# hsinnan75/GSAlign

Hardware: AMD Instinct MI355X
Metric: aligned query Gbp/s (whole node) (higher is better)
Workload: dtype u8; 1 GPU; full-human-sized pair (BASELINE configs[4]): 24 contigs with GRCh38 chromosome lengths, 3.08 Gbp, repeat injection, vs 1; inflight_contexts_per_gpu=8, world_size=1, parallelism=one GPU

## Files before the change

### gsalign_amd/csrc/gsa_api.hip

```cpp
#include <algorithm>
#include <atomic>
#include <chrono>
#include <cstring>
#include <mutex>
#include <thread>
#include <pthread.h>
#include <sched.h>
#include "gsa_ctx.h"

static thread_local std::string g_create_error;

int gsa_fail(gsa_ctx *ctx, int code, const std::string &msg)
{
	if (ctx) ctx->err = msg; else g_create_error = msg;
	return code;
}

int host_stage4_5_6(gsa_ctx *c, int stage);
int host_stage8_finish(gsa_ctx *c);
int build_block_view(gsa_ctx *c);
void bundle_split_lists(gsa_ctx *c);
void bundle_join_lists(gsa_ctx *c);

void collect_events(gsa_ctx *c)
// ... 418 lines not shown
	return GSA_OK;
}

int gsa_set_option(gsa_ctx *c, const char *name, int64_t value)
{
	if (!c || !name) return GSA_ERR_ARG;
	const std::string k(name);
	auto in = [&](int64_t lo, int64_t hi) { return value >= lo && value <= hi; };
	const int64_t BIG = (int64_t)1 << 40;
	if (k == "split_min") { if (!in(0, BIG)) return gsa_fail(c, GSA_ERR_ARG, "split_min: 0 .. 2^40 bases"); c->opt.split_min = value; }
	else if (k == "bundle_contig") { if (!in(0, BIG)) return gsa_fail(c, GSA_ERR_ARG, "bundle_contig: 0 (no bundles) .. 2^40 bases"); c->opt.bundle_contig = value; }
	else if (k == "bundle_cap") { if (!in(1, BIG)) return gsa_fail(c, GSA_ERR_ARG, "bundle_cap: 1 .. 2^40 bases"); c->opt.bundle_cap = value; }
	else if (k == "seed_budget") { if (!in(1, 0xffffffffll)) return gsa_fail(c, GSA_ERR_ARG, "seed_budget: 1 .. 2^32 - 1 wave-iterations"); c->seed_budget = (u32)value; }
	else if (k == "dp_lane") { if (!in(0, 1 << 20)) return gsa_fail(c, GSA_ERR_ARG, "dp_lane: 0 (round 2's tiny / small split) .. 2^20 cells"); c->opt.dp_lane = (int)value; }
	else if (k == "seed_mode") { if (value < 0 || value > 2) return gsa_fail(c, GSA_ERR_ARG, "seed_mode: 0 sweep, 1 speculative, 2 search"); c->opt.seed_mode = (int)value; }
	else if (k == "pd_bitmap") c->opt.pd_bitmap = value != 0;
	else if (k == "dp_side") c->opt.dp_side = value != 0;
	else if (k == "dp_small_side") c->opt.dp_small_side = value != 0;
	else if (k == "pd_two_level_min") { if (!in(0, BIG)) return gsa_fail(c, GSA_ERR_ARG, "pd_two_level_min: >= 0 blocks"); c->opt.pd_two_level_min = value; }
	else if (k == "dp_occupancy") { if (!in(0, 16)) return gsa_fail(c, GSA_ERR_ARG, "dp_occupancy: 0 (off) .. 16 workgroups per CU"); c->opt.dp_occupancy = (int)value; }
	else if (k == "pd_bytes") { if (!in(0, 2)) return gsa_fail(c, GSA_ERR_ARG, "pd_bytes: 0 never, 1 by the hit count, 2 always"); c->opt.pd_bytes = (int)value; }
	else if (k == "pres_from_kmer") c->opt.pres_from_kmer = value != 0;
	else if (k == "walk_chain_min") { if (!in(0, BIG)) return gsa_fail(c, GSA_ERR_ARG, "walk_chain_min: >= 0 seeds"); c->opt.walk_chain_min = value; }
	else if (k == "sweep_shape") { if (value < -1 || value > 1) return gsa_fail(c, GSA_ERR_ARG, "sweep_shape: -1, 0 or 1"); c->opt.sweep_shape = (int)value; }
	else if (k == "dp_safe") c->dp_safe = value != 0;
	else if (k == "dp_fake_timeout") { if (!in(0, 1 << 20)) return gsa_fail(c, GSA_ERR_ARG, "dp_fake_timeout: >= 0"); c->dp_fake_timeout = (int)value; }
	else return gsa_fail(c, GSA_ERR_ARG, "gsa_set_option: unknown option " + k);
	return GSA_OK;
}

// ... 732 lines not shown
```

### gsalign_amd/csrc/gsa_ctx.h

```cpp
#ifndef GSA_CTX_H
#define GSA_CTX_H
#include <atomic>
#include <chrono>
#include <condition_variable>
#include <deque>
#include <mutex>
#include <thread>
#include "gsa_internal.h"

struct Leaf {
	i32 beg, end;
	i32 sumlen;
	i32 q_first, q_last_end;
	i64 r_first, r_last_end;
	i32 blk;
	i32 cut4, cut5;
	i32 blk_score;
};

enum { M_NB = 0, M_NC = 1, M_NBLK = 2, M_NG = 3, M_NR = 4, M_NJ = 5, M_NL = 6, M_LBERR = 7, M_ANY = 8, M_NTINY = 40, M_TICKET = 48, M_NBRAW = 49, M_NR2 = 50, M_NF = 51, M_NJOB = 52, M_OPSTOT = 53, M_NALN = 54, M_DPERR = 64, M_NLARGE = 65, M_DPERR2 = 66, M_CELLS = 68  , M_DPERR3 = 41, M_LBDONE = 42, M_LFSTEPS = 44 , M_NEARLY = 62, M_EOPS = 63, M_NTOUCH = 46 , M_MAXBLK = 56 , MAIL_N = 72 };
#define LEAF_CHUNK 1024

struct HostBlock {
	i32 leaf_beg, leaf_end;
// ... 18 lines not shown
	struct Piece { void *dst; const void *src; size_t n; };
	struct Job { std::vector<Piece> pieces; std::atomic<int> *busy; std::atomic<int> *err; std::chrono::steady_clock::time_point t_push; };
	double copy_ms = 0, wait_ms = 0, bytes = 0; long long jobs = 0;
	int device = 0; hipStream_t st = nullptr;
	std::thread th; std::mutex mu; std::condition_variable cv; std::deque<Job> q; bool stop = false;
	size_t n_demand = 0;
	void run();
	void push(Job &&j) { j.busy->fetch_add(1); j.t_push = std::chrono::steady_clock::now(); { std::lock_guard<std::mutex> g(mu); q.push_back(std::move(j)); } cv.notify_one(); }
};

struct Options {
	int64_t split_min = 20000000;
	int64_t bundle_contig = 16000000;
	int64_t bundle_cap = 64000000;
	int dp_lane = 512;
	int seed_mode = 1;
	int pd_bitmap = 1;
	int sweep_shape = -1;
	int dp_small_side = 0;
	int dp_side = 0;
	int64_t walk_chain_min = 100000;
	int64_t pd_two_level_min = 2000000;
	int dp_occupancy = 0;
	int pd_bytes = 1;
	int pres_from_kmer = 1;
	int kmer_k = 0;
};

struct gsa_ctx {
	int device = 0;
// ... 203 lines not shown
```

### gsalign_amd/csrc/k_seed.hip

```cpp
#include <cstring>
#include <mutex>
#include <condition_variable>
#include <vector>
#include "gsa_ctx.h"
#include "gsa_fm.h"
#include "gsa_scan.h"

enum { CNT_OCCBLK = 0, CNT_DONE = 1, CNT_HITS = 2, CNT_SEEDS = 3, CNT_DPCELLS = 4, CNT_DPJOBS = 5, CNT_DPMN = 6, CNT_CAND = 8, CNT_OVERFLOW = 9, CNT_OCCBLK_ALL = 10, CNT_HEAVY = 12 };

#ifndef SEED_WG
#define SEED_WG 64
#endif
#ifndef NSUB
#define NSUB 96
#endif
#ifndef ADV_STEPS
#define ADV_STEPS 4
#endif
#ifndef PLOOK
#define PLOOK 3
#endif
#define PATH_WORDS 320
#define QP_WORDS (GSA_CHUNK / 16 + 4)
#define QN_WORDS (GSA_CHUNK / 32 + 4)
enum { M_DONE = 0, M_FM = 1, M_TEXT = 2, M_KMER = 3, M_LOC = 4, M_ADV = 5, M_KLO = 6, M_MLOC = 7, M_MTEXT = 8 };
#ifndef SEED_MULTI
#define SEED_MULTI 1
#endif

__device__ __forceinline__ int q_code(const u32 *qp, int p) { return (qp[p >> 4] >> ((p & 15) << 1)) & 3; }
__device__ __forceinline__ int q_isn(const u32 *qn, int p) { return (qn[p >> 5] >> (p & 31)) & 1; }
__device__ __forceinline__ u64 funnel64(u32 w0, u32 w1, u32 w2, int sh)
{
	const u64 lo = (u64)w0 | ((u64)w1 << 32);
	return sh ? (lo >> sh) | ((u64)w2 << (64 - sh)) : lo;
}
__device__ __forceinline__ u64 q_bits64(const u32 *qp, int p) { const int w = p >> 4; return funnel64(qp[w], qp[w + 1], qp[w + 2], (p & 15) << 1); }
__device__ __forceinline__ u32 q_nbits32(const u32 *qn, int p) { const int w = p >> 5; return (u32)((((u64)qn[w + 1] << 32) | qn[w]) >> (p & 31)); }

__device__ __forceinline__ int text_match32(u32 r0, u32 r1, u32 r2, i64 tp, i64 tend, const u32 *qp, const u32 *qn, int pos, int clen)
{
	int avail = clen - pos;
	if (tend - tp < (i64)avail) avail = (int)(tend - tp);
	if (avail > 32) avail = 32;
	if (avail <= 0) return 0;
	const u64 d = funnel64(r0, r1, r2, (int)(tp & 15) << 1) ^ q_bits64(qp, pos);
	const u64 dm = (d | (d >> 1)) & 0x5555555555555555ull;
	const u32 nm = q_nbits32(qn, pos);
	int n = dm ? (__ffsll((unsigned long long)dm) - 1) >> 1 : 32;
	const int fn = nm ? __ffs((int)nm) - 1 : 32;
	n = n < fn ? n : fn;
	return n < avail ? n : avail;
}

__device__ __forceinline__ u32 pres4_line(u64 qb, int K) { return (u32)((qb >> 6) & ((1ull << (2 * (K - 3))) - 1)); }
__device__ __forceinline__ u32 pres4_bit(u64 qb, int K, int i)
{
	const u32 head = (u32)(qb >> (2 * i)) & ((1u << (2 * (3 - i))) - 1);
	const u32 tail = (u32)(qb >> (2 * K)) & ((1u << (2 * i)) - 1);
	return (u32)i * 64u + (head | (tail << (2 * (3 - i))));
}

template <int TPB>
// ... 36 lines not shown
		for (int k = 0; k < V; k++) { const int idx = b0 + lane * V + k; v[k] = idx < n1 ? __hip_atomic_load(&hits[idx], __ATOMIC_RELAXED, __HIP_MEMORY_SCOPE_AGENT) : 0; }
#pragma unroll
		for (int k = 0; k < V; k++) tsum += v[k];
		i32 inc = tsum;
		for (int o = 1; o < 64; o <<= 1) { const i32 t = __shfl_up(inc, o); if (lane >= o) inc += t; }
		i32 e = run + inc - tsum;
#pragma unroll
		for (int k = 0; k < V; k++) { const int idx = b0 + lane * V + k; if (idx < n1) base[idx] = e; e += v[k]; }
		run += __shfl(inc, 63);
	}
}

#ifndef SEED_MIN_WAVES
#define SEED_MIN_WAVES 5
#endif
#ifndef LHOP_N
#define LHOP_N 1024
#endif
#define MEMO_WORDS (GSA_CHUNK / 16)
__device__ __forceinline__ int memo_nib(const u32 *memo, int s) { return (int)((memo[s >> 4] >> ((s & 15) << 1)) & 3u); }
__device__ __forceinline__ void memo_one(u32 *memo, int s) { atomicOr(&memo[s >> 4], 1u << ((s & 15) << 1)); }
__device__ __forceinline__ int memo_get(const u32 *memo, const u32 *lhop, int s)
{
	const int v = memo_nib(memo, s);
	if (v < 2) return v;
	if (v == 2) return 5;
	for (u32 h = ((u32)s * 40503u) >> 6;; h++) { const u32 e = lhop[h & (LHOP_N - 1)]; if ((e >> 16) == (u32)s + 1) return (int)(e & 0xffffu); }
}
__device__ __forceinline__ void memo_set(u32 *memo, u32 *lhop, int s, int d, int *abort_flag)
{
	if (d == 1 || d == 5) { atomicOr(&memo[s >> 4], (d == 1 ? 1u : 2u) << ((s & 15) << 1)); return; }
	const u32 e = ((u32)(s + 1) << 16) | (u32)d;
	u32 h = ((u32)s * 40503u) >> 6;
	for (int tries = 0; tries < LHOP_N; tries++, h++) {
		const u32 old = atomicCAS(&lhop[h & (LHOP_N - 1)], 0u, e);
		if (old == 0 || old == e) { atomicOr(&memo[s >> 4], 3u << ((s & 15) << 1)); return; }
	}
	*(volatile int *)abort_flag = 1;
}

__device__ __forceinline__ u32 nt4_quad(u32 w)
{
	const u32 l = w | 0x20202020u;
	const u32 x = (l >> 1) & 0x03030303u;
	u32 code = x ^ ((x >> 1) & 0x01010101u);
	const u32 want = __builtin_amdgcn_perm(0u, 0x74676361u, code);
	const u32 diff = l ^ want;
	const u32 bad = ((diff | ((diff & 0x7f7f7f7fu) + 0x7f7f7f7fu)) >> 7) & 0x01010101u;
	code &= ~(bad * 3u);
	return ((code * 0x01041040u) >> 24) | (((bad * 0x01020408u) >> 24) & 15u) << 8;
// ... 9 lines not shown
	}
	w0 = w1 = wn = 0;
#pragma unroll
	for (int t = 0; t < 8; t++) {
		const u32 r = nt4_quad(d[t]);
		if (t < 4) w0 |= (r & 0xffu) << (8 * t); else w1 |= (r & 0xffu) << (8 * (t - 4));
		wn |= (r >> 8) << (4 * t);
	}
}

template <bool COUNT, int NCH>
struct SeedLds {
	static constexpr int NV = NCH * NSUB;
	u32 s_ncand[NCH], s_queue, s_hits[NCH];
	int changed, s_abort;
	u32 qp[NCH][QP_WORDS], qn[NCH][QN_WORDS];
	u32 memo[NCH][MEMO_WORDS];
	u32 lhop[NCH][LHOP_N];
	uint16_t mblk[COUNT ? GSA_CHUNK : 1];
	u32 bits[NCH][PATH_WORDS];
	uint16_t entry_of[NV], exit_of[NV];
	uint16_t pend_it[SEED_WG];
	uint16_t jmp[2][NV], walked_from[NV];
	u32 rewalked[(NV + 31) / 32], onchain[(NV + 31) / 32], s_npend;
	int s_last;
};
#define SEED_SYNC() do { if (WPW == 1) __syncthreads(); else { __builtin_amdgcn_fence(__ATOMIC_RELEASE, "wavefront"); __builtin_amdgcn_wave_barrier(); __builtin_amdgcn_fence(__ATOMIC_ACQUIRE, "wavefront"); } } while (0)
#define s_ncand sl_.s_ncand
#define s_queue sl_.s_queue
#define s_hits sl_.s_hits
#define changed sl_.changed
#define s_abort sl_.s_abort
#define qp sl_.qp
#define qn sl_.qn
#define memo sl_.memo
#define lhop sl_.lhop
#define mblk sl_.mblk
#define bits sl_.bits
#define entry_of sl_.entry_of
#define exit_of sl_.exit_of
#define pend_it sl_.pend_it
#define jmp sl_.jmp
#define walked_from sl_.walked_from
#define rewalked sl_.rewalked
#define onchain sl_.onchain
#define s_npend sl_.s_npend
#define s_last sl_.s_last
template <bool COUNT, bool E16, int NCH, int WPW>
__device__ __forceinline__ void seed_chunk(const DevIndex &di, const uint8_t *__restrict__ q, i32 qlen, const Params &prm, u64 *cnt,
                                                      i32 *cand_s, i32 *cand_len, u64 *cand_x0, i32 *cand_freq, u32 cand_cap, u32 *cand_cnt, u32 *onpath, i32 *chunk_hits, u64 *hcnt,
                                                      u32 budget, u32 *heavy_list, i32 *chunk_base, const int chunk0, const u32 n_chunks, SeedLds<COUNT, NCH> &sl_)
{
	constexpr int NV = NCH * NSUB;
	static_assert(!COUNT || NCH == 1, "the accounting build walks one chunk per wave");
	const int j = threadIdx.x & 63;
	const int nch = (u32)chunk0 + NCH <= n_chunks ? NCH : (int)(n_chunks - (u32)chunk0);
	i64 c0[NCH]; int clen[NCH], S[NCH], nitems[NCH]; size_t cbase[NCH];
#pragma unroll
	for (int ch = 0; ch < NCH; ch++) {
		c0[ch] = (i64)(chunk0 + ch) * GSA_CHUNK;
		clen[ch] = ch < nch ? (int)((i64)qlen - c0[ch] < GSA_CHUNK ? (i64)qlen - c0[ch] : GSA_CHUNK) : 0;
		S[ch] = (clen[ch] + NSUB - 1) / NSUB; if (S[ch] < 1) S[ch] = 1;
		nitems[ch] = (clen[ch] + S[ch] - 1) / S[ch];
		cbase[ch] = (size_t)(chunk0 + ch) * cand_cap;
	}
	const int nitems_all = NCH == 1 ? nitems[0] : nitems[0] + nitems[NCH - 1];
#define CH_SEL(ARR, CH) (NCH == 1 ? ARR[0] : ((CH) ? ARR[NCH - 1] : ARR[0]))
#pragma unroll
	for (int ch = 0; ch < NCH; ch++) {
		for (int g = j; g < QN_WORDS; g += SEED_WG) {
			u32 w0 = 0, w1 = 0, wn = 0;
			const int p0 = g << 5;
			if (p0 < clen[ch]) stage32(q + c0[ch] + p0, p0, clen[ch], w0, w1, wn);
			if (2 * g < QP_WORDS) qp[ch][2 * g] = w0;
			if (2 * g + 1 < QP_WORDS) qp[ch][2 * g + 1] = w1;
			qn[ch][g] = wn;
		}
		for (int p = j; p < MEMO_WORDS; p += SEED_WG) memo[ch][p] = 0;
		for (int p = j; p < LHOP_N; p += SEED_WG) lhop[ch][p] = 0;
		for (int p = j; p < PATH_WORDS; p += SEED_WG) bits[ch][p] = 0;
		for (int it = j; it < nitems[ch]; it += SEED_WG) entry_of[ch * NSUB + it] = (uint16_t)(it * S[ch]);
		if (j == 0) { s_ncand[ch] = 0; s_hits[ch] = 0; }
	}
	if (j == 0) { s_queue = 0; s_npend = 0; s_abort = 0; }
	if (j < (NV + 31) / 32) rewalked[j] = 0;
	u32 all_blocks = 0, rounds = 0, iters = 0;
#ifdef SEED_STATS
	u32 st_it = 0, st_fm_any = 0, st_fm_only = 0, st_act = 0, st_fm = 0;
#endif
	unsigned long long t_begin = wall_clock64(), t_round0 = 0, t_resolve = 0;
	u32 dirty = 0;
	int fb_item = 0;
	SEED_SYNC();
	for (;;) {
		int item = -1, s = 0, bend = 0, pos = 0, mode = M_ADV; u32 kid = 0, pid = 0, pext = 0;
		int lclen = 0;
		const u32 *qp_l = qp[0], *qn_l = qn[0]; u32 *memo_l = memo[0], *lhop_l = lhop[0];
		FmIntv ik = {0, 0, 0}; u32 blk = 0; i64 tp = 0;
		i64 mp[4] = {0, 0, 0, 0}; u32 malive = 0;
		bool need_item = true;
		while (!__all(mode == M_DONE)) {
			iters++;
			if (!COUNT && budget && iters > budget) *(volatile int *)&s_abort = 1;
			if (*(volatile int *)&s_abort) break;
#ifdef SEED_STATS
			{ const u64 bf = __ballot(mode == M_FM), ba = __ballot(mode != M_DONE);
			  st_it++; st_fm_any += bf != 0; st_fm_only += bf != 0 && bf == ba; st_act += __popcll(ba); st_fm += __popcll(bf); }
#endif
			u64 kk = 0, ll = 0; bool kn = true, ln = true;
			if (mode == M_FM) {
				const u64 k = ik.x1 - 1, l = ik.x1 - 1 + ik.x2;
				kn = (k == (u64)-1); ln = (l == (u64)-1);
// ... 34 lines not shown
				if (__any(mode == M_MTEXT)) {
					const bool mt = mode == M_MTEXT;
					w5b = *(const W5 *)(di.ref2 + ((mt && (malive & 2u)) ? (mp[1] >> 4) : 0));
					w5c = *(const W5 *)(di.ref2 + ((mt && (malive & 4u)) ? (mp[2] >> 4) : 0));
					w5d = *(const W5 *)(di.ref2 + ((mt && (malive & 8u)) ? (mp[3] >> 4) : 0));
				}
			}
			bool ended = false;
			if (mode == M_KMER) {
				if (!PRES4_TEST(0)) {
					memo_one(memo_l, s); s += 1; mode = M_ADV;
					const int L = prm.MinSeedLength < 32 ? prm.MinSeedLength : 32;
#pragma unroll
					for (int k2 = 0; k2 < PLOOK; k2++) {
						if (s >= bend || memo_nib(memo_l, s)) break;
						const u32 nb = q_nbits32(qn_l, s);
						if (s + prm.MinSeedLength > lclen || (nb & (L == 32 ? ~0u : (1u << L) - 1)) != 0) break;
						if (k2 == 0 ? PRES4_TEST(1) : k2 == 1 ? PRES4_TEST(2) : PRES4_TEST(3)) break;
						memo_one(memo_l, s); s += 1;
					}
				} else {
					const bool hit = e1.x != 0;
					if (hit) { ik.x0 = e0.x; ik.x1 = e0.y; ik.x2 = e1.x; pos = s + di.kmer_k; }
					else ik = fm_init(di, q_code(qp_l, s));
					mode = M_FM;
					if (hit && ik.x2 == 1) { tp = (i64)(e1.y - 1) + di.kmer_k; mode = M_TEXT; }
					else if (!COUNT && SEED_MULTI > 1 && hit && ik.x2 <= SEED_MULTI) mode = M_MLOC;
				}
			} else if (mode == M_LOC) {
				tp = (i64)sav + (pos - s); mode = M_TEXT;
			} else if (!COUNT && SEED_MULTI > 1 && mode == M_MLOC) {
				mp[0] = (i64)sav + (pos - s); mp[1] = (i64)sav1 + (pos - s); mp[2] = (i64)sav2 + (pos - s); mp[3] = (i64)sav3 + (pos - s);
				malive = (1u << (int)ik.x2) - 1u; mode = M_MTEXT;
			} else if (!COUNT && SEED_MULTI > 1 && mode == M_MTEXT) {
				int g0 = -1, g1 = -1, g2 = -1, g3 = -1;
#define MT_ROW(G, W, P) { int got = text_match32(W.a, W.b, W.c, P, (i64)di.seq_len, qp_l, qn_l, pos, lclen); if (got == 32) got += text_match32(W.c, W.d, W.e, P + 32, (i64)di.seq_len, qp_l, qn_l, pos + 32, lclen); G = got; }
				if (malive & 1u) MT_ROW(g0, w5, mp[0])
				if (malive & 2u) MT_ROW(g1, w5b, mp[1])
				if (malive & 4u) MT_ROW(g2, w5c, mp[2])
				if (malive & 8u) MT_ROW(g3, w5d, mp[3])
#undef MT_ROW
				int m = g0 > g1 ? g0 : g1; m = m > g2 ? m : g2; m = m > g3 ? m : g3;
				const u32 na = (g0 == m ? 1u : 0u) | (g1 == m ? 2u : 0u) | (g2 == m ? 4u : 0u) | (g3 == m ? 8u : 0u);
				pos += m; mp[0] += m; mp[1] += m; mp[2] += m; mp[3] += m;
				if (m < 64 || __popc(na) == 1) {
					const int first = __ffs((int)na) - 1;
					ik.x0 += (u64)first; ik.x2 = (u64)__popc(na);
					if (m == 64) { tp = first == 0 ? mp[0] : first == 1 ? mp[1] : first == 2 ? mp[2] : mp[3]; mode = M_TEXT; }
					else ended = true;
				} else malive = na;
				if (mode == M_MTEXT && !ended && malive != na) malive = na;
			} else if (mode == M_TEXT) {
				int got = text_match32(r0, r1, r2, tp, (i64)di.seq_len, qp_l, qn_l, pos, lclen);
				if (got == 32) got += text_match32(r2, r3, r4, tp + 32, (i64)di.seq_len, qp_l, qn_l, pos + 32, lclen);
				pos += got; tp += got;
				ended = got < 64;
			} else if (mode == M_FM) {
				const bool can = pos < lclen && !q_isn(qn_l, pos < lclen ? pos : 0);
				const bool ok = can && fm_extend_loaded(di, ik, q_code(qp_l, pos < lclen ? pos : 0), bk, bl, kk, ll, kn, ln, blk);
				ended = !ok;
				if (ok) { pos++; if (!COUNT && ik.x2 == 1) mode = M_LOC; else if (!COUNT && SEED_MULTI > 1 && ik.x2 <= SEED_MULTI) mode = M_MLOC; }
			}
			if (ended) {
				const int len = pos - s;
				int d = 1;
				if (len >= prm.MinSeedLength && ik.x2 <= GSA_MAX_SEED_FREQ) {
					const int ch = NCH == 1 ? 0 : (item >= NSUB ? NCH - 1 : 0);
					const u32 slot = atomicAdd(&s_ncand[ch], 1u);
					const size_t cb = CH_SEL(cbase, ch);
					if (slot < cand_cap) { cand_s[cb + slot] = (i32)(CH_SEL(c0, ch) + s); cand_len[cb + slot] = len; cand_x0[cb + slot] = ik.x0; cand_freq[cb + slot] = (i32)ik.x2; }
					else cnt[CNT_OVERFLOW] = 1;
					d = prm.bSensitive ? 5 : len + 1;
				}
				memo_set(memo_l, lhop_l, s, d, &s_abort); if (COUNT) mblk[s] = (uint16_t)blk;
				all_blocks += blk;
				s += d; mode = M_ADV;
			}
			for (int step = 0; step < ADV_STEPS && mode == M_ADV; step++) {
				if (need_item) {
					if (rounds == 0) {
						const u32 it_ = atomicAdd(&s_queue, 1u);
						if (NCH == 1) item = it_ < (u32)nitems[0] ? (int)it_ : -1;
						else {
							const u32 both = 2u * (u32)(nitems[0] < nitems[NCH - 1] ? nitems[0] : nitems[NCH - 1]);
							if (it_ < both) item = (int)(it_ >> 1) + ((it_ & 1u) ? NSUB : 0);
							else if (it_ < (u32)nitems_all) { const int r = (int)(it_ - both) + (int)(both >> 1); item = nitems[0] > nitems[NCH - 1] ? r : NSUB + r; }
							else item = -1;
						}
					}
					else if (dirty) { dirty = 0; item = fb_item; }
					else item = -1;
					need_item = false;
					if (item < 0) { mode = M_DONE; break; }
					const int ch = NCH == 1 ? 0 : (item >= NSUB ? NCH - 1 : 0), li = item - ch * NSUB;
					lclen = CH_SEL(clen, ch); qp_l = qp[ch]; qn_l = qn[ch]; memo_l = memo[ch]; lhop_l = lhop[ch];
					const int S_l = CH_SEL(S, ch);
					s = entry_of[item]; bend = (li + 1) * S_l < lclen ? (li + 1) * S_l : lclen;
				}
				if (s >= bend) { exit_of[item] = (uint16_t)s; need_item = true; continue; }
				const int m_ = memo_get(memo_l, lhop_l, s);
				if (m_) { s += m_; continue; }
				const u32 nb = q_nbits32(qn_l, s);
				const int L = prm.MinSeedLength < 32 ? prm.MinSeedLength : 32;
				if (nb & 1u) { memo_one(memo_l, s); if (COUNT) mblk[s] = 0; s += 1; }
				else if (!COUNT && (s + prm.MinSeedLength > lclen || (nb & (L == 32 ? ~0u : (1u << L) - 1)) != 0)) { memo_one(memo_l, s); s += 1; }
				else {
					pos = s + 1; blk = 0; mode = M_FM;
#ifdef SEED_EAGER_INIT
					ik = fm_init(di, q_code(qp_l, s));
#endif
					if (COUNT || !(di.kmer_k > 1 && s + di.kmer_k <= lclen && (nb & ((1u << di.kmer_k) - 1)) == 0)) ik = fm_init(di, q_code(qp_l, s));
					else {
						const u64 qb = q_bits64(qp_l, s);
						kid = (u32)(qb & ((1ull << (2 * di.kmer_k)) - 1)); mode = M_KMER;
						pid = di.pres_k ? pres4_line(qb, di.pres_k) : 0;
						pext = di.pres_k ? (((u32)qb & 63u) | (((u32)(qb >> (2 * di.pres_k)) & 63u) << 6)) : 0;
					}
// ... 50 lines not shown
		t_resolve += wall_clock64() - t_r0;
		const int again = changed;
		if (again && j < (int)s_npend) { fb_item = pend_it[j]; dirty = 1; }
		SEED_SYNC();
		if (!again) break;
	}
	const bool heavy = s_abort != 0;
	if (heavy) {
		if (j == 0) for (int ch = 0; ch < nch; ch++) {
			const u32 hslot = (u32)atomicAdd((unsigned long long *)&cnt[CNT_HEAVY], 1ull);
			heavy_list[hslot] = (u32)(chunk0 + ch);
			s_ncand[ch] = 0; cand_cnt[chunk0 + ch] = 0; lb_pub(&chunk_hits[chunk0 + ch], 0); if (chunk0 + ch == 0) lb_pub(&chunk_hits[n_chunks], 0);
		}
		SEED_SYNC();
	}
	u32 alg_blocks = 0;
	if (!heavy) for (int v = j; v < NV; v += SEED_WG) if (V_LIVE(v)) {
		const int ch = v >= NSUB ? NCH - 1 : 0, li = v - ch * NSUB;
		const int bend = (li + 1) * CH_SEL(S, ch) < CH_SEL(clen, ch) ? (li + 1) * CH_SEL(S, ch) : CH_SEL(clen, ch);
		for (int s = entry_of[v]; s < bend;) { atomicOr(&bits[ch][s >> 5], 1u << (s & 31)); if (COUNT) alg_blocks += mblk[s]; s += memo_get(memo[ch], lhop[ch], s); }
	}
#undef V_LIVE
	for (int o = 32; o; o >>= 1) { alg_blocks += __shfl_down(alg_blocks, o); all_blocks += __shfl_down(all_blocks, o); }
	if ((j & 63) == 0) {
		if (alg_blocks) atomicAdd((unsigned long long *)&cnt[CNT_OCCBLK], (unsigned long long)alg_blocks);
		if (all_blocks) atomicAdd((unsigned long long *)&cnt[CNT_OCCBLK_ALL], (unsigned long long)all_blocks);
#ifndef SEED_STATS
		atomicMax((unsigned long long *)&cnt[13], (unsigned long long)iters);
#endif
	}
#ifdef SEED_STATS
	if ((j & 63) == 0) { atomicAdd((unsigned long long *)&cnt[11], (unsigned long long)st_it); atomicAdd((unsigned long long *)&cnt[13], (unsigned long long)st_fm_any); atomicAdd((unsigned long long *)&cnt[14], (unsigned long long)st_fm_only);
	                     atomicAdd((unsigned long long *)&cnt[15], (unsigned long long)st_act); atomicAdd((unsigned long long *)&cnt[7], (unsigned long long)st_fm); }
	if (false)
#endif
// ... 4 lines not shown
		for (int ch = 0; ch < NCH; ch++) if (ch < nch) {
			for (int p = j; p < PATH_WORDS; p += SEED_WG) onpath[(size_t)(chunk0 + ch) * PATH_WORDS + p] = bits[ch][p];
			const u32 nc = s_ncand[ch] < cand_cap ? s_ncand[ch] : cand_cap;
			u32 h = 0;
			for (u32 i = j; i < nc; i += SEED_WG) { const i32 p = cand_s[cbase[ch] + i] - (i32)c0[ch]; if ((bits[ch][p >> 5] >> (p & 31)) & 1u) h += (u32)cand_freq[cbase[ch] + i]; }
			for (int o = 32; o; o >>= 1) h += __shfl_down(h, o);
			if ((j & 63) == 0 && h) atomicAdd(&s_hits[ch], h);
		}
		SEED_SYNC();
		if (j == 0) for (int ch = 0; ch < nch; ch++) {
			const u32 nc = s_ncand[ch] < cand_cap ? s_ncand[ch] : cand_cap;
			cand_cnt[chunk0 + ch] = nc; lb_pub(&chunk_hits[chunk0 + ch], (i32)s_hits[ch]); if (chunk0 + ch == 0) lb_pub(&chunk_hits[n_chunks], 0); atomicMax((unsigned long long *)&cnt[CNT_CAND], (unsigned long long)s_ncand[ch]);
			if (s_hits[ch]) atomicAdd((unsigned long long *)&cnt[CNT_HITS], (unsigned long long)s_hits[ch]);
		}
	}
#undef CH_SEL
	asm volatile("s_waitcnt vmcnt(0)" ::: "memory");
	SEED_SYNC();
	if (j == 0) {
		__builtin_amdgcn_fence(__ATOMIC_RELEASE, "workgroup");
		s_last = atomicAdd((unsigned long long *)&cnt[CNT_DONE], (unsigned long long)nch) == (unsigned long long)n_chunks - (unsigned long long)nch ? 1 : 0;
	}
	SEED_SYNC();
	if (s_last && j < 16) {
		hcnt[j] = j == CNT_DONE ? 0 : __hip_atomic_load(&cnt[j], __ATOMIC_RELAXED, __HIP_MEMORY_SCOPE_AGENT);
		cnt[j] = 0;
	}
	if (s_last) { if (WPW == 1) wg_exscan_hits<SEED_WG>(chunk_hits, chunk_base, (int)n_chunks + 1); else wave_exscan_hits(chunk_hits, chunk_base, (int)n_chunks + 1); }
}
#undef s_ncand
#undef s_queue
#undef s_hits
#undef changed
#undef s_abort
#undef qp
#undef qn
#undef memo
#undef lhop
#undef mblk
#undef bits
#undef entry_of
#undef exit_of
#undef pend_it
#undef jmp
#undef walked_from
#undef rewalked
#undef onchain
#undef s_npend
#undef s_last
#undef SEED_SYNC


#define SEED_TICKET 16
#ifndef SEED_PERSIST
#define SEED_PERSIST 12
#endif
#ifndef SEED_NCH
#define SEED_NCH 1
#endif
#ifndef SEED_WPW
#define SEED_WPW 8
#endif
#ifndef SEED_WGS_PER_CU
#define SEED_WGS_PER_CU 1
#endif
#define SEED_WG_LDS_MIN ((160 * 1024) / (SEED_WGS_PER_CU + 1) + 2048)
#define SEED_LB_WAVES(COUNT_) ((COUNT_) ? 1 : SEED_MIN_WAVES)
template <bool COUNT, bool E16>
__global__ void __launch_bounds__(SEED_WG * (COUNT ? 1 : SEED_WPW), SEED_LB_WAVES(COUNT)) k_seed_wg(DevIndex di, const uint8_t *__restrict__ q, i32 qlen, Params prm, u64 *cnt,
                                                      i32 *cand_s, i32 *cand_len, u64 *cand_x0, i32 *cand_freq, u32 cand_cap, u32 *cand_cnt, u32 *onpath, i32 *chunk_hits, u64 *hcnt,
                                                      u32 budget, u32 *heavy_list, i32 *chunk_base, u64 tk_base, u32 n_chunks)
{
	constexpr int NCH = COUNT ? 1 : SEED_NCH;
	constexpr int WPW = COUNT ? 1 : SEED_WPW;
	typedef SeedLds<COUNT, NCH> Lds;
	extern __shared__ __attribute__((aligned(16))) unsigned char seed_dyn_lds[];
	Lds *lds = (Lds *)seed_dyn_lds;
	Lds &L = lds[WPW == 1 ? 0 : (threadIdx.x >> 6)];
	for (;;) {
		u32 unit = 0;
		if ((threadIdx.x & 63) == 0) unit = (u32)(atomicAdd((unsigned long long *)&cnt[SEED_TICKET], 1ull) - tk_base);
		unit = (u32)__builtin_amdgcn_readfirstlane((int)unit);
		if ((u64)unit * NCH >= n_chunks) return;
		seed_chunk<COUNT, E16, NCH, WPW>(di, q, qlen, prm, cnt, cand_s, cand_len, cand_x0, cand_freq, cand_cap, cand_cnt, onpath, chunk_hits, hcnt, budget, heavy_list, chunk_base, (int)(unit * NCH), n_chunks, L);
	}
}


#define DENSE_TPB 256
#define DENSE_WGS(SPAN) ((GSA_CHUNK + (SPAN) - 1) / (SPAN))
template <bool E16, int DENSE_SPAN>
__global__ void __launch_bounds__(DENSE_TPB) k_dense_search(DevIndex di, const uint8_t *__restrict__ q, i32 qlen, Params prm, const u32 *__restrict__ chunk_list,
                                                              u32 *dn_lf, u64 *dn_x0, u64 *cnt)
{
	__shared__ u32 qp[QP_WORDS], qn[QN_WORDS];
	const u32 slot = blockIdx.x / DENSE_WGS(DENSE_SPAN), part = blockIdx.x % DENSE_WGS(DENSE_SPAN);
	const u32 chunk = chunk_list ? chunk_list[slot] : slot;
	const int j = threadIdx.x;
	const i64 c0 = (i64)chunk * GSA_CHUNK;
// ... 978 lines not shown
		u64 hits = 0, maxcand = 0, n_heavy = dense_all ? (u64)n_chunks : 0;
		occ_all = 0;
		if (!dense_all) {
#define GSA_SEED_ARGS c->di, d_q, qlen, c->prm, cnt, c->d_cand_s.as<i32>(), c->d_cand_len.as<i32>(), c->d_cand_x0.as<u64>(), c->d_cand_freq.as<i32>(), (u32)ccap, \
			c->d_cand_cnt.as<u32>(), c->d_onpath.as<u32>(), c->d_chunk_hits.as<i32>(), c->h_cnt, budget, c->d_heavy.as<u32>(), c->d_chunk_base.as<i32>()
			const i64 n_units = c->count_blocks ? n_chunks : (n_chunks + SEED_NCH - 1) / SEED_NCH;
			const int wpw = c->count_blocks ? 1 : SEED_WPW;
			unsigned grid = (unsigned)((n_units + wpw - 1) / wpw);
			if (!c->count_blocks) {
				if (c->n_cus <= 0) { hipDeviceProp_t pr; GSA_CHECK(c, hipGetDeviceProperties(&pr, c->device)); c->n_cus = pr.multiProcessorCount; }
				const i64 cap = (i64)c->n_cus * (SEED_WPW > 1 ? SEED_WGS_PER_CU : SEED_PERSIST);
				if (cap < (i64)grid) grid = (unsigned)cap;
			}
			const u64 tk_base = c->seed_ticket; c->seed_ticket += (u64)n_units + (u64)grid * (u64)wpw;
			const size_t dl_count = sizeof(SeedLds<true, 1>);
			size_t dl = sizeof(SeedLds<false, SEED_NCH>) * SEED_WPW; if (SEED_WPW > 1 && dl < SEED_WG_LDS_MIN) dl = SEED_WG_LDS_MIN;
			if (c->count_blocks) hipLaunchKernelGGL((k_seed_wg<true, false>), dim3(grid), dim3(SEED_WG), dl_count, st, GSA_SEED_ARGS, tk_base, (u32)n_chunks);
			else if (c->di.kmer_e16) hipLaunchKernelGGL((k_seed_wg<false, true>), dim3(grid), dim3(SEED_WG * SEED_WPW), dl, st, GSA_SEED_ARGS, tk_base, (u32)n_chunks);
			else hipLaunchKernelGGL((k_seed_wg<false, false>), dim3(grid), dim3(SEED_WG * SEED_WPW), dl, st, GSA_SEED_ARGS, tk_base, (u32)n_chunks);
#undef GSA_SEED_ARGS
			if (c->profiling || c->prof_seed) hipEventRecord(c->ev[1], st);
			GSA_CHECK(c, hipEventRecord(c->ev[21], st));
			GSA_CHECK(c, hipEventSynchronize(c->ev[21]));
			hits = c->h_cnt[CNT_HITS]; maxcand = c->h_cnt[CNT_CAND]; n_heavy = c->h_cnt[CNT_HEAVY]; occ_all = c->h_cnt[CNT_OCCBLK_ALL];
			c->dbg[0] = c->h_cnt[11]; c->dbg[1] = n_heavy; c->dbg[2] = c->h_cnt[13]; c->dbg[3] = c->h_cnt[14]; c->dbg[4] = c->h_cnt[15]; c->dbg[5] = c->h_cnt[7];
			c->counters[0] = c->h_cnt[CNT_OCCBLK];
			if (seed_mode == 1) {
				c->seed_sweep_next = n_heavy * 5 > (u64)n_chunks * 2;
				c->seed_sweep_period = (c->seed_sweep_next && c->seed_sweep_probe) ? (c->seed_sweep_period < 64 ? c->seed_sweep_period * 2 : 64) : 8;
				c->seed_sweep_probe = false;
			}
		}
		if (n_heavy > 0) {
			const size_t nd = (size_t)n_heavy * GSA_CHUNK;
// ... 182 lines not shown
```

Measured before the change: 33.39 Gbp/s.

## Shrink seed kernel LDS by aliasing N-mask and path bitmap into existing tables

Removes the per-chunk qn and bits arrays from the seed kernel's LDS. The N-mask now lives in the tail of the long-hop table, and the on-path bitmap reuses the query words after the walk finishes. An optional diet mode (off by default) shrinks the long-hop table, skips N checks for chunks with no N, and packs 12 waves per workgroup. With the default settings the per-wave LDS footprint shrinks while the workgroup LDS is pinned at 100 KiB, so occupancy stays the same and the gain would mostly come from less zero-initialisation. It also adds a seed_lhop option to cap the hash table's size.

```diff
diff --git a/gsalign_amd/csrc/gsa_api.hip b/gsalign_amd/csrc/gsa_api.hip
--- a/gsalign_amd/csrc/gsa_api.hip
+++ b/gsalign_amd/csrc/gsa_api.hip
@@ -456,6 +456,7 @@
 	else if (k == "seed_budget") { if (!in(1, 0xffffffffll)) return gsa_fail(c, GSA_ERR_ARG, "seed_budget: 1 .. 2^32 - 1 wave-iterations"); c->seed_budget = (u32)value; }
 	else if (k == "dp_lane") { if (!in(0, 1 << 20)) return gsa_fail(c, GSA_ERR_ARG, "dp_lane: 0 (round 2's tiny / small split) .. 2^20 cells"); c->opt.dp_lane = (int)value; }
 	else if (k == "seed_mode") { if (value < 0 || value > 2) return gsa_fail(c, GSA_ERR_ARG, "seed_mode: 0 sweep, 1 speculative, 2 search"); c->opt.seed_mode = (int)value; }
+	else if (k == "seed_lhop") { if (value != 0 && (!in(16, 1 << 16) || (value & (value - 1)))) return gsa_fail(c, GSA_ERR_ARG, "seed_lhop: 0 or a power of two >= 16"); c->opt.seed_lhop = (int)value; }
 	else if (k == "pd_bitmap") c->opt.pd_bitmap = value != 0;
 	else if (k == "dp_side") c->opt.dp_side = value != 0;
 	else if (k == "dp_small_side") c->opt.dp_small_side = value != 0;
diff --git a/gsalign_amd/csrc/gsa_ctx.h b/gsalign_amd/csrc/gsa_ctx.h
--- a/gsalign_amd/csrc/gsa_ctx.h
+++ b/gsalign_amd/csrc/gsa_ctx.h
@@ -56,6 +56,7 @@
 	int64_t bundle_contig = 16000000;
 	int64_t bundle_cap = 64000000;
 	int dp_lane = 512;
+	int seed_lhop = 0;
 	int seed_mode = 1;
 	int pd_bitmap = 1;
 	int sweep_shape = -1;
diff --git a/gsalign_amd/csrc/k_seed.hip b/gsalign_amd/csrc/k_seed.hip
--- a/gsalign_amd/csrc/k_seed.hip
+++ b/gsalign_amd/csrc/k_seed.hip
@@ -29,16 +29,16 @@
 #endif
 
 __device__ __forceinline__ int q_code(const u32 *qp, int p) { return (qp[p >> 4] >> ((p & 15) << 1)) & 3; }
-__device__ __forceinline__ int q_isn(const u32 *qn, int p) { return (qn[p >> 5] >> (p & 31)) & 1; }
+__device__ __forceinline__ int q_isn(const u32 *qn, int p, bool on = true) { return on ? (qn[p >> 5] >> (p & 31)) & 1 : 0; }
 __device__ __forceinline__ u64 funnel64(u32 w0, u32 w1, u32 w2, int sh)
 {
 	const u64 lo = (u64)w0 | ((u64)w1 << 32);
 	return sh ? (lo >> sh) | ((u64)w2 << (64 - sh)) : lo;
 }
 __device__ __forceinline__ u64 q_bits64(const u32 *qp, int p) { const int w = p >> 4; return funnel64(qp[w], qp[w + 1], qp[w + 2], (p & 15) << 1); }
-__device__ __forceinline__ u32 q_nbits32(const u32 *qn, int p) { const int w = p >> 5; return (u32)((((u64)qn[w + 1] << 32) | qn[w]) >> (p & 31)); }
-
-__device__ __forceinline__ int text_match32(u32 r0, u32 r1, u32 r2, i64 tp, i64 tend, const u32 *qp, const u32 *qn, int pos, int clen)
+__device__ __forceinline__ u32 q_nbits32(const u32 *qn, int p, bool on = true) { if (!on) return 0u; const int w = p >> 5; return (u32)((((u64)qn[w + 1] << 32) | qn[w]) >> (p & 31)); }
+
+__device__ __forceinline__ int text_match32(u32 r0, u32 r1, u32 r2, i64 tp, i64 tend, const u32 *qp, const u32 *qn, int pos, int clen, bool qn_on = true)
 {
 	int avail = clen - pos;
 	if (tend - tp < (i64)avail) avail = (int)(tend - tp);
@@ -46,7 +46,7 @@
 	if (avail <= 0) return 0;
 	const u64 d = funnel64(r0, r1, r2, (int)(tp & 15) << 1) ^ q_bits64(qp, pos);
 	const u64 dm = (d | (d >> 1)) & 0x5555555555555555ull;
-	const u32 nm = q_nbits32(qn, pos);
+	const u32 nm = q_nbits32(qn, pos, qn_on);
 	int n = dm ? (__ffsll((unsigned long long)dm) - 1) >> 1 : 32;
 	const int fn = nm ? __ffs((int)nm) - 1 : 32;
 	n = n < fn ? n : fn;
@@ -113,26 +113,34 @@
 #ifndef SEED_MIN_WAVES
 #define SEED_MIN_WAVES 5
 #endif
+#ifndef SEED_LDS_DIET
+#define SEED_LDS_DIET 0
+#endif
 #ifndef LHOP_N
-#define LHOP_N 1024
-#endif
+#define LHOP_N (SEED_LDS_DIET ? 512 : 1024)
+#endif
+#ifndef LHOP_NN
+#define LHOP_NN (SEED_LDS_DIET ? 256 : LHOP_N)
+#endif
+#define LHOP_WORDS (LHOP_NN + QN_WORDS > LHOP_N ? LHOP_NN + QN_WORDS : LHOP_N)
+static_assert((LHOP_N & (LHOP_N - 1)) == 0 && (LHOP_NN & (LHOP_NN - 1)) == 0 && LHOP_NN <= LHOP_N, "the long-hop table is indexed with a mask");
 #define MEMO_WORDS (GSA_CHUNK / 16)
 __device__ __forceinline__ int memo_nib(const u32 *memo, int s) { return (int)((memo[s >> 4] >> ((s & 15) << 1)) & 3u); }
 __device__ __forceinline__ void memo_one(u32 *memo, int s) { atomicOr(&memo[s >> 4], 1u << ((s & 15) << 1)); }
-__device__ __forceinline__ int memo_get(const u32 *memo, const u32 *lhop, int s)
+__device__ __forceinline__ int memo_get(const u32 *memo, const u32 *lhop, u32 lmask, int s)
 {
 	const int v = memo_nib(memo, s);
 	if (v < 2) return v;
 	if (v == 2) return 5;
-	for (u32 h = ((u32)s * 40503u) >> 6;; h++) { const u32 e = lhop[h & (LHOP_N - 1)]; if ((e >> 16) == (u32)s + 1) return (int)(e & 0xffffu); }
-}
-__device__ __forceinline__ void memo_set(u32 *memo, u32 *lhop, int s, int d, int *abort_flag)
+	for (u32 h = ((u32)s * 40503u) >> 6;; h++) { const u32 e = lhop[h & lmask]; if ((e >> 16) == (u32)s + 1) return (int)(e & 0xffffu); }
+}
+__device__ __forceinline__ void memo_set(u32 *memo, u32 *lhop, u32 lmask, int s, int d, int *abort_flag)
 {
 	if (d == 1 || d == 5) { atomicOr(&memo[s >> 4], (d == 1 ? 1u : 2u) << ((s & 15) << 1)); return; }
 	const u32 e = ((u32)(s + 1) << 16) | (u32)d;
 	u32 h = ((u32)s * 40503u) >> 6;
-	for (int tries = 0; tries < LHOP_N; tries++, h++) {
-		const u32 old = atomicCAS(&lhop[h & (LHOP_N - 1)], 0u, e);
+	for (u32 tries = 0; tries <= lmask; tries++, h++) {
+		const u32 old = atomicCAS(&lhop[h & lmask], 0u, e);
 		if (old == 0 || old == e) { atomicOr(&memo[s >> 4], 3u << ((s & 15) << 1)); return; }
 	}
 	*(volatile int *)abort_flag = 1;
@@ -172,11 +180,10 @@
 	static constexpr int NV = NCH * NSUB;
 	u32 s_ncand[NCH], s_queue, s_hits[NCH];
 	int changed, s_abort;
-	u32 qp[NCH][QP_WORDS], qn[NCH][QN_WORDS];
+	u32 qp[NCH][QP_WORDS];
 	u32 memo[NCH][MEMO_WORDS];
-	u32 lhop[NCH][LHOP_N];
+	u32 lhop[NCH][LHOP_WORDS];
 	uint16_t mblk[COUNT ? GSA_CHUNK : 1];
-	u32 bits[NCH][PATH_WORDS];
 	uint16_t entry_of[NV], exit_of[NV];
 	uint16_t pend_it[SEED_WG];
 	uint16_t jmp[2][NV], walked_from[NV];
@@ -190,11 +197,9 @@
 #define changed sl_.changed
 #define s_abort sl_.s_abort
 #define qp sl_.qp
-#define qn sl_.qn
 #define memo sl_.memo
 #define lhop sl_.lhop
 #define mblk sl_.mblk
-#define bits sl_.bits
 #define entry_of sl_.entry_of
 #define exit_of sl_.exit_of
 #define pend_it sl_.pend_it
@@ -207,7 +212,7 @@
 template <bool COUNT, bool E16, int NCH, int WPW>
 __device__ __forceinline__ void seed_chunk(const DevIndex &di, const uint8_t *__restrict__ q, i32 qlen, const Params &prm, u64 *cnt,
                                                       i32 *cand_s, i32 *cand_len, u64 *cand_x0, i32 *cand_freq, u32 cand_cap, u32 *cand_cnt, u32 *onpath, i32 *chunk_hits, u64 *hcnt,
-                                                      u32 budget, u32 *heavy_list, i32 *chunk_base, const int chunk0, const u32 n_chunks, SeedLds<COUNT, NCH> &sl_)
+                                                      u32 budget, u32 *heavy_list, i32 *chunk_base, const int chunk0, const u32 n_chunks, const u32 lhop_cap, SeedLds<COUNT, NCH> &sl_)
 {
 	constexpr int NV = NCH * NSUB;
 	static_assert(!COUNT || NCH == 1, "the accounting build walks one chunk per wave");
@@ -226,20 +231,29 @@
 #define CH_SEL(ARR, CH) (NCH == 1 ? ARR[0] : ((CH) ? ARR[NCH - 1] : ARR[0]))
 #pragma unroll
 	for (int ch = 0; ch < NCH; ch++) {
+		for (int p = j; p < MEMO_WORDS; p += SEED_WG) memo[ch][p] = 0;
+		for (int p = j; p < LHOP_WORDS; p += SEED_WG) lhop[ch][p] = 0;
+		for (int it = j; it < nitems[ch]; it += SEED_WG) entry_of[ch * NSUB + it] = (uint16_t)(it * S[ch]);
+		if (j == 0) { s_ncand[ch] = 0; s_hits[ch] = 0; }
+	}
+	SEED_SYNC();
+	int hasn[NCH];
+#pragma unroll
+	for (int ch = 0; ch < NCH; ch++) {
+		bool anyn = false;
 		for (int g = j; g < QN_WORDS; g += SEED_WG) {
 			u32 w0 = 0, w1 = 0, wn = 0;
 			const int p0 = g << 5;
 			if (p0 < clen[ch]) stage32(q + c0[ch] + p0, p0, clen[ch], w0, w1, wn);
 			if (2 * g < QP_WORDS) qp[ch][2 * g] = w0;
 			if (2 * g + 1 < QP_WORDS) qp[ch][2 * g + 1] = w1;
-			qn[ch][g] = wn;
-		}
-		for (int p = j; p < MEMO_WORDS; p += SEED_WG) memo[ch][p] = 0;
-		for (int p = j; p < LHOP_N; p += SEED_WG) lhop[ch][p] = 0;
-		for (int p = j; p < PATH_WORDS; p += SEED_WG) bits[ch][p] = 0;
-		for (int it = j; it < nitems[ch]; it += SEED_WG) entry_of[ch * NSUB + it] = (uint16_t)(it * S[ch]);
-		if (j == 0) { s_ncand[ch] = 0; s_hits[ch] = 0; }
-	}
+			if (p0 + 32 > clen[ch]) wn = p0 < clen[ch] ? wn & ((1u << (clen[ch] - p0)) - 1u) : 0u;
+			if (wn) { lhop[ch][LHOP_NN + g] = wn; anyn = true; }
+		}
+		hasn[ch] = !SEED_LDS_DIET || __any(anyn) ? 1 : 0;
+	}
+#define QN_OF(CH) ((const u32 *)&lhop[CH][LHOP_NN])
+#define LMASK_OF(CH) ((SEED_LDS_DIET && CH_SEL(hasn, CH) && lhop_cap > (u32)LHOP_NN ? (u32)LHOP_NN : lhop_cap) - 1u)
 	if (j == 0) { s_queue = 0; s_npend = 0; s_abort = 0; }
 	if (j < (NV + 31) / 32) rewalked[j] = 0;
 	u32 all_blocks = 0, rounds = 0, iters = 0;
@@ -253,7 +267,7 @@
 	for (;;) {
 		int item = -1, s = 0, bend = 0, pos = 0, mode = M_ADV; u32 kid = 0, pid = 0, pext = 0;
 		int lclen = 0;
-		const u32 *qp_l = qp[0], *qn_l = qn[0]; u32 *memo_l = memo[0], *lhop_l = lhop[0];
+		const u32 *qp_l = qp[0], *qn_l = QN_OF(0); u32 *memo_l = memo[0], *lhop_l = lhop[0]; u32 lmask_l = LMASK_OF(0); bool hasn_l = CH_SEL(hasn, 0) != 0;
 		FmIntv ik = {0, 0, 0}; u32 blk = 0; i64 tp = 0;
 		i64 mp[4] = {0, 0, 0, 0}; u32 malive = 0;
 		bool need_item = true;
@@ -318,7 +332,7 @@
 #pragma unroll
 					for (int k2 = 0; k2 < PLOOK; k2++) {
 						if (s >= bend || memo_nib(memo_l, s)) break;
-						const u32 nb = q_nbits32(qn_l, s);
+						const u32 nb = q_nbits32(qn_l, s, hasn_l);
 						if (s + prm.MinSeedLength > lclen || (nb & (L == 32 ? ~0u : (1u << L) - 1)) != 0) break;
 						if (k2 == 0 ? PRES4_TEST(1) : k2 == 1 ? PRES4_TEST(2) : PRES4_TEST(3)) break;
 						memo_one(memo_l, s); s += 1;
@@ -338,7 +352,7 @@
 				malive = (1u << (int)ik.x2) - 1u; mode = M_MTEXT;
 			} else if (!COUNT && SEED_MULTI > 1 && mode == M_MTEXT) {
 				int g0 = -1, g1 = -1, g2 = -1, g3 = -1;
-#define MT_ROW(G, W, P) { int got = text_match32(W.a, W.b, W.c, P, (i64)di.seq_len, qp_l, qn_l, pos, lclen); if (got == 32) got += text_match32(W.c, W.d, W.e, P + 32, (i64)di.seq_len, qp_l, qn_l, pos + 32, lclen); G = got; }
+#define MT_ROW(G, W, P) { int got = text_match32(W.a, W.b, W.c, P, (i64)di.seq_len, qp_l, qn_l, pos, lclen, hasn_l); if (got == 32) got += text_match32(W.c, W.d, W.e, P + 32, (i64)di.seq_len, qp_l, qn_l, pos + 32, lclen, hasn_l); G = got; }
 				if (malive & 1u) MT_ROW(g0, w5, mp[0])
 				if (malive & 2u) MT_ROW(g1, w5b, mp[1])
 				if (malive & 4u) MT_ROW(g2, w5c, mp[2])
@@ -355,12 +369,12 @@
 				} else malive = na;
 				if (mode == M_MTEXT && !ended && malive != na) malive = na;
 			} else if (mode == M_TEXT) {
-				int got = text_match32(r0, r1, r2, tp, (i64)di.seq_len, qp_l, qn_l, pos, lclen);
-				if (got == 32) got += text_match32(r2, r3, r4, tp + 32, (i64)di.seq_len, qp_l, qn_l, pos + 32, lclen);
+				int got = text_match32(r0, r1, r2, tp, (i64)di.seq_len, qp_l, qn_l, pos, lclen, hasn_l);
+				if (got == 32) got += text_match32(r2, r3, r4, tp + 32, (i64)di.seq_len, qp_l, qn_l, pos + 32, lclen, hasn_l);
 				pos += got; tp += got;
 				ended = got < 64;
 			} else if (mode == M_FM) {
-				const bool can = pos < lclen && !q_isn(qn_l, pos < lclen ? pos : 0);
+				const bool can = pos < lclen && !q_isn(qn_l, pos < lclen ? pos : 0, hasn_l);
 				const bool ok = can && fm_extend_loaded(di, ik, q_code(qp_l, pos < lclen ? pos : 0), bk, bl, kk, ll, kn, ln, blk);
 				ended = !ok;
 				if (ok) { pos++; if (!COUNT && ik.x2 == 1) mode = M_LOC; else if (!COUNT && SEED_MULTI > 1 && ik.x2 <= SEED_MULTI) mode = M_MLOC; }
@@ -376,7 +390,7 @@
 					else cnt[CNT_OVERFLOW] = 1;
 					d = prm.bSensitive ? 5 : len + 1;
 				}
-				memo_set(memo_l, lhop_l, s, d, &s_abort); if (COUNT) mblk[s] = (uint16_t)blk;
+				memo_set(memo_l, lhop_l, lmask_l, s, d, &s_abort); if (COUNT) mblk[s] = (uint16_t)blk;
 				all_blocks += blk;
 				s += d; mode = M_ADV;
 			}
@@ -397,14 +411,14 @@
 					need_item = false;
 					if (item < 0) { mode = M_DONE; break; }
 					const int ch = NCH == 1 ? 0 : (item >= NSUB ? NCH - 1 : 0), li = item - ch * NSUB;
-					lclen = CH_SEL(clen, ch); qp_l = qp[ch]; qn_l = qn[ch]; memo_l = memo[ch]; lhop_l = lhop[ch];
+					lclen = CH_SEL(clen, ch); qp_l = qp[ch]; qn_l = QN_OF(ch); memo_l = memo[ch]; lhop_l = lhop[ch]; lmask_l = LMASK_OF(ch); hasn_l = CH_SEL(hasn, ch) != 0;
 					const int S_l = CH_SEL(S, ch);
 					s = entry_of[item]; bend = (li + 1) * S_l < lclen ? (li + 1) * S_l : lclen;
 				}
 				if (s >= bend) { exit_of[item] = (uint16_t)s; need_item = true; continue; }
-				const int m_ = memo_get(memo_l, lhop_l, s);
+				const int m_ = memo_get(memo_l, lhop_l, lmask_l, s);
 				if (m_) { s += m_; continue; }
-				const u32 nb = q_nbits32(qn_l, s);
+				const u32 nb = q_nbits32(qn_l, s, hasn_l);
 				const int L = prm.MinSeedLength < 32 ? prm.MinSeedLength : 32;
 				if (nb & 1u) { memo_one(memo_l, s); if (COUNT) mblk[s] = 0; s += 1; }
 				else if (!COUNT && (s + prm.MinSeedLength > lclen || (nb & (L == 32 ? ~0u : (1u << L) - 1)) != 0)) { memo_one(memo_l, s); s += 1; }
@@ -485,11 +499,18 @@
 		}
 		SEED_SYNC();
 	}
+	static_assert(PATH_WORDS <= QP_WORDS, "the on-path bitmap lies in the query's words");
+#define bits qp
 	u32 alg_blocks = 0;
+	if (!heavy) {
+#pragma unroll
+		for (int ch = 0; ch < NCH; ch++) for (int p = j; p < PATH_WORDS; p += SEED_WG) bits[ch][p] = 0;
+		SEED_SYNC();
+	}
 	if (!heavy) for (int v = j; v < NV; v += SEED_WG) if (V_LIVE(v)) {
 		const int ch = v >= NSUB ? NCH - 1 : 0, li = v - ch * NSUB;
 		const int bend = (li + 1) * CH_SEL(S, ch) < CH_SEL(clen, ch) ? (li + 1) * CH_SEL(S, ch) : CH_SEL(clen, ch);
-		for (int s = entry_of[v]; s < bend;) { atomicOr(&bits[ch][s >> 5], 1u << (s & 31)); if (COUNT) alg_blocks += mblk[s]; s += memo_get(memo[ch], lhop[ch], s); }
+		for (int s = entry_of[v]; s < bend;) { atomicOr(&bits[ch][s >> 5], 1u << (s & 31)); if (COUNT) alg_blocks += mblk[s]; s += memo_get(memo[ch], lhop[ch], LMASK_OF(ch), s); }
 	}
 #undef V_LIVE
 	for (int o = 32; o; o >>= 1) { alg_blocks += __shfl_down(alg_blocks, o); all_blocks += __shfl_down(all_blocks, o); }
@@ -524,6 +545,9 @@
 			if (s_hits[ch]) atomicAdd((unsigned long long *)&cnt[CNT_HITS], (unsigned long long)s_hits[ch]);
 		}
 	}
+#undef bits
+#undef QN_OF
+#undef LMASK_OF
 #undef CH_SEL
 	asm volatile("s_waitcnt vmcnt(0)" ::: "memory");
 	SEED_SYNC();
@@ -544,11 +568,9 @@
 #undef changed
 #undef s_abort
 #undef qp
-#undef qn
 #undef memo
 #undef lhop
 #undef mblk
-#undef bits
 #undef entry_of
 #undef exit_of
 #undef pend_it
@@ -569,21 +591,27 @@
 #define SEED_NCH 1
 #endif
 #ifndef SEED_WPW
-#define SEED_WPW 8
+#define SEED_WPW (SEED_LDS_DIET ? 12 : 8)
 #endif
 #ifndef SEED_WGS_PER_CU
 #define SEED_WGS_PER_CU 1
 #endif
 #define SEED_WG_LDS_MIN ((160 * 1024) / (SEED_WGS_PER_CU + 1) + 2048)
+#ifndef SEED_WG_LDS
+#define SEED_WG_LDS 102400
+#endif
+static_assert(SEED_WPW == 1 || (SEED_WG_LDS >= SEED_WG_LDS_MIN && SEED_WG_LDS <= 160 * 1024), "a fat workgroup's LDS: more than half a CU's, so that two never share one");
 #define SEED_LB_WAVES(COUNT_) ((COUNT_) ? 1 : SEED_MIN_WAVES)
 template <bool COUNT, bool E16>
 __global__ void __launch_bounds__(SEED_WG * (COUNT ? 1 : SEED_WPW), SEED_LB_WAVES(COUNT)) k_seed_wg(DevIndex di, const uint8_t *__restrict__ q, i32 qlen, Params prm, u64 *cnt,
                                                       i32 *cand_s, i32 *cand_len, u64 *cand_x0, i32 *cand_freq, u32 cand_cap, u32 *cand_cnt, u32 *onpath, i32 *chunk_hits, u64 *hcnt,
-                                                      u32 budget, u32 *heavy_list, i32 *chunk_base, u64 tk_base, u32 n_chunks)
+                                                      u32 budget, u32 *heavy_list, i32 *chunk_base, u64 tk_base, u32 n_chunks, u32 lhop_cap)
 {
 	constexpr int NCH = COUNT ? 1 : SEED_NCH;
 	constexpr int WPW = COUNT ? 1 : SEED_WPW;
 	typedef SeedLds<COUNT, NCH> Lds;
+	static_assert(WPW == 1 || sizeof(Lds) * WPW <= SEED_WG_LDS, "SeedLds has outgrown the workgroup's LDS: SEED_WPW waves no longer fit SEED_WG_LDS bytes");
+	static_assert(sizeof(Lds) % 4 == 0, "one SeedLds per wave, back to back");
 	extern __shared__ __attribute__((aligned(16))) unsigned char seed_dyn_lds[];
 	Lds *lds = (Lds *)seed_dyn_lds;
 	Lds &L = lds[WPW == 1 ? 0 : (threadIdx.x >> 6)];
@@ -592,7 +620,7 @@
 		if ((threadIdx.x & 63) == 0) unit = (u32)(atomicAdd((unsigned long long *)&cnt[SEED_TICKET], 1ull) - tk_base);
 		unit = (u32)__builtin_amdgcn_readfirstlane((int)unit);
 		if ((u64)unit * NCH >= n_chunks) return;
-		seed_chunk<COUNT, E16, NCH, WPW>(di, q, qlen, prm, cnt, cand_s, cand_len, cand_x0, cand_freq, cand_cap, cand_cnt, onpath, chunk_hits, hcnt, budget, heavy_list, chunk_base, (int)(unit * NCH), n_chunks, L);
+		seed_chunk<COUNT, E16, NCH, WPW>(di, q, qlen, prm, cnt, cand_s, cand_len, cand_x0, cand_freq, cand_cap, cand_cnt, onpath, chunk_hits, hcnt, budget, heavy_list, chunk_base, (int)(unit * NCH), n_chunks, lhop_cap, L);
 	}
 }
 
@@ -1601,10 +1629,11 @@
 			}
 			const u64 tk_base = c->seed_ticket; c->seed_ticket += (u64)n_units + (u64)grid * (u64)wpw;
 			const size_t dl_count = sizeof(SeedLds<true, 1>);
-			size_t dl = sizeof(SeedLds<false, SEED_NCH>) * SEED_WPW; if (SEED_WPW > 1 && dl < SEED_WG_LDS_MIN) dl = SEED_WG_LDS_MIN;
-			if (c->count_blocks) hipLaunchKernelGGL((k_seed_wg<true, false>), dim3(grid), dim3(SEED_WG), dl_count, st, GSA_SEED_ARGS, tk_base, (u32)n_chunks);
-			else if (c->di.kmer_e16) hipLaunchKernelGGL((k_seed_wg<false, true>), dim3(grid), dim3(SEED_WG * SEED_WPW), dl, st, GSA_SEED_ARGS, tk_base, (u32)n_chunks);
-			else hipLaunchKernelGGL((k_seed_wg<false, false>), dim3(grid), dim3(SEED_WG * SEED_WPW), dl, st, GSA_SEED_ARGS, tk_base, (u32)n_chunks);
+			size_t dl = sizeof(SeedLds<false, SEED_NCH>) * SEED_WPW; if (SEED_WPW > 1 && dl < SEED_WG_LDS) dl = SEED_WG_LDS;
+			const u32 lhop_cap = c->opt.seed_lhop > 0 && c->opt.seed_lhop < LHOP_N ? (u32)c->opt.seed_lhop : (u32)LHOP_N;
+			if (c->count_blocks) hipLaunchKernelGGL((k_seed_wg<true, false>), dim3(grid), dim3(SEED_WG), dl_count, st, GSA_SEED_ARGS, tk_base, (u32)n_chunks, lhop_cap);
+			else if (c->di.kmer_e16) hipLaunchKernelGGL((k_seed_wg<false, true>), dim3(grid), dim3(SEED_WG * SEED_WPW), dl, st, GSA_SEED_ARGS, tk_base, (u32)n_chunks, lhop_cap);
+			else hipLaunchKernelGGL((k_seed_wg<false, false>), dim3(grid), dim3(SEED_WG * SEED_WPW), dl, st, GSA_SEED_ARGS, tk_base, (u32)n_chunks, lhop_cap);
 #undef GSA_SEED_ARGS
 			if (c->profiling || c->prof_seed) hipEventRecord(c->ev[1], st);
 			GSA_CHECK(c, hipEventRecord(c->ev[21], st));
```

Result: faster. 33.88 Gbp/s (median of 6 runs) (+1.5%).
